# crowsonkb/style_transfer2

Hardware: AMD Instinct MI355X
Metric: style-transfer iters/sec @1024px VGG19 (higher is better)
Workload: dtype f32; 1 GPU; configs[1]: 1024x1024 single image per GPU, VGG19 to conv5_1, content conv4_2 + 5 style layers, adam fp32, 500 iterations per image; jobs=1, parallelism=independent jobs, 1 per GPU, no collective (replicas)

## Files before the change

style_transfer2_amd/csrc/gram.hip:

```cpp
#include "st2_kernels.h"
#include "env.h"
#include "wave_reduce.h"
#include <stdint.h>
#include <stdlib.h>

namespace st2 {

typedef float f32x16 __attribute__((ext_vector_type(16)));

constexpr int GKT = 32;
constexpr int GLD = GKT + 1;

GramPlan gram_plan(int C, int hw)
{
    GramPlan p;
    p.bt = C > 64 ? 128 : 64;
    const int t = (C + p.bt - 1) / p.bt;
    p.tiles = t * (t + 1) / 2;
    const int target128 = (int)env_int("ST2_GRAM_BLOCKS", 512), target64 = (int)env_int("ST2_GRAM_BLOCKS64", 1024);
    int want = p.bt == 128 ? target128 / p.tiles : (target64 + p.tiles - 1) / p.tiles;
    const int max_splits = (hw + 4 * GKT - 1) / (4 * GKT);
    if (want > max_splits) want = max_splits;
    if (want < 1) want = 1;
    int kslab = (hw + want - 1) / want;
// ... 88 lines not shown
            for (int i = 0; i < T; ++i)
#pragma unroll
                for (int j = 0; j < T; ++j)
                    acc[i][j] = __builtin_amdgcn_mfma_f32_32x32x2f32(av[i], bv[j], acc[i][j], 0, 0, 0);
        }
    }

    float* dst = slabs + (size_t)split * C * C;
#pragma unroll
    for (int i = 0; i < T; ++i)
#pragma unroll
        for (int j = 0; j < T; ++j) {
            const int col = j0 + wn * (T * 32) + j * 32 + l31;
#pragma unroll
            for (int e = 0; e < 16; ++e) {
                const int row = i0 + wm * (T * 32) + i * 32 + (e & 3) + 8 * (e >> 2) + 4 * khalf;
                if (row < C && col < C) dst[(size_t)row * C + col] = acc[i][j][e];
            }
        }
}

typedef __attribute__((address_space(3))) void* gram_lptr_t;
typedef float gf32x4 __attribute__((ext_vector_type(4)));

template <int BT>
__device__ __forceinline__ void gram_partial_dma_body(const float* __restrict__ F, unsigned f_bytes, float* __restrict__ slabs,
                                                      int C, int hw, int tiles_1d, int kslab)
{
    constexpr int T = BT / 64;
    constexpr int IMG = BT * 32;
    constexpr int PIECES = IMG / 256;
    constexpr int PPW = PIECES / 4;
    __shared__ __attribute__((aligned(16))) float smem[2][2][IMG];

    const int tid = threadIdx.x, lane = tid & 63;
    const int wave = __builtin_amdgcn_readfirstlane(tid >> 6);
    const int wm = wave >> 1, wn = wave & 1;
    const int n_ut = tiles_1d * (tiles_1d + 1) / 2;
    int tile = blockIdx.x % n_ut;
    const int split = blockIdx.x / n_ut;
    int ti = 0;
    while (tile >= tiles_1d - ti) { tile -= tiles_1d - ti; ++ti; }
    const int tj = ti + tile;
    const int i0 = ti * BT, j0 = tj * BT;
    const bool diag = ti == tj;
    const int kbeg = split * kslab;
    const int kend = min(hw, kbeg + kslab);
    const int nsteps = (kend - kbeg) / 32;

    const __amdgpu_buffer_rsrc_t rs = __builtin_amdgcn_make_buffer_rsrc((void*)F, 0, f_bytes, 0x00020000);
    unsigned aoff[PPW], boff[PPW];
#pragma unroll
    for (int t = 0; t < PPW; ++t) {
        const int slot = (wave + 4 * t) * 64 + lane;
        const int r = slot >> 3, q = (slot & 7) ^ ((r >> 1) & 7);
        aoff[t] = i0 + r < C ? ((unsigned)(i0 + r) * (unsigned)hw + (unsigned)kbeg + 4u * q) * 4u : 0xffffffffu;
        boff[t] = j0 + r < C ? ((unsigned)(j0 + r) * (unsigned)hw + (unsigned)kbeg + 4u * q) * 4u : 0xffffffffu;
    }
    auto dma = [&](int step, int stage) {
        const unsigned so = (unsigned)step * 128u;
#pragma unroll
        for (int t = 0; t < PPW; ++t) {
            __builtin_amdgcn_raw_ptr_buffer_load_lds(rs, (gram_lptr_t)(smem[stage][0] + (wave + 4 * t) * 256), 16,
                                                     aoff[t] == 0xffffffffu ? aoff[t] : aoff[t] + so, 0, 0, 0);
            if (!diag)
                __builtin_amdgcn_raw_ptr_buffer_load_lds(rs, (gram_lptr_t)(smem[stage][1] + (wave + 4 * t) * 256), 16,
                                                         boff[t] == 0xffffffffu ? boff[t] : boff[t] + so, 0, 0, 0);
        }
    };

    f32x16 acc[T][T];
#pragma unroll
    for (int i = 0; i < T; ++i)
#pragma unroll
        for (int j = 0; j < T; ++j)
#pragma unroll
            for (int e = 0; e < 16; ++e) acc[i][j][e] = 0.f;

    const int l31 = lane & 31;
    const bool hi = lane >= 32;
    int arow[T], brow[T];
#pragma unroll
    for (int i = 0; i < T; ++i) { arow[i] = wm * (T * 32) + i * 32 + l31; brow[i] = wn * (T * 32) + i * 32 + l31; }

    if (nsteps > 0) dma(0, 0);
    for (int st = 0; st < nsteps; ++st) {
        const int cur = st & 1;
        asm volatile("s_waitcnt vmcnt(0)" ::: "memory");
        __syncthreads();
        if (st + 1 < nsteps) dma(st + 1, cur ^ 1);
        const float* As = smem[cur][0];
        const float* Bs = diag ? smem[cur][0] : smem[cur][1];
#pragma unroll
        for (int q = 0; q < 8; ++q) {
            float a0[T], a1[T], b0[T], b1[T];
#pragma unroll
            for (int i = 0; i < T; ++i) {
                const gf32x4 v = *reinterpret_cast<const gf32x4*>(As + (arow[i] * 8 + (q ^ ((arow[i] >> 1) & 7))) * 4);
                a0[i] = hi ? v.y : v.x; a1[i] = hi ? v.w : v.z;
            }
#pragma unroll
            for (int j = 0; j < T; ++j) {
                const gf32x4 v = *reinterpret_cast<const gf32x4*>(Bs + (brow[j] * 8 + (q ^ ((brow[j] >> 1) & 7))) * 4);
                b0[j] = hi ? v.y : v.x; b1[j] = hi ? v.w : v.z;
            }
#pragma unroll
            for (int i = 0; i < T; ++i)
#pragma unroll
                for (int j = 0; j < T; ++j) {
                    acc[i][j] = __builtin_amdgcn_mfma_f32_32x32x2f32(a0[i], b0[j], acc[i][j], 0, 0, 0);
                    acc[i][j] = __builtin_amdgcn_mfma_f32_32x32x2f32(a1[i], b1[j], acc[i][j], 0, 0, 0);
                }
        }
    }

    const int khalf = lane >> 5;
    float* dst = slabs + (size_t)split * C * C;
#pragma unroll
    for (int i = 0; i < T; ++i)
#pragma unroll
        for (int j = 0; j < T; ++j) {
            const int col = j0 + wn * (T * 32) + j * 32 + l31;
#pragma unroll
            for (int e = 0; e < 16; ++e) {
                const int row = i0 + wm * (T * 32) + i * 32 + (e & 3) + 8 * (e >> 2) + 4 * khalf;
                if (row < C && col < C) dst[(size_t)row * C + col] = acc[i][j][e];
            }
        }
}

__global__ __launch_bounds__(256, 2) void gram_partial_dma_128(const float* F, unsigned f_bytes, float* slabs, int C, int hw, int tiles_1d, int kslab)
{ gram_partial_dma_body<128>(F, f_bytes, slabs, C, hw, tiles_1d, kslab); }
__global__ __launch_bounds__(256, 2) void gram_partial_dma_64(const float* F, unsigned f_bytes, float* slabs, int C, int hw, int tiles_1d, int kslab)
{ gram_partial_dma_body<64>(F, f_bytes, slabs, C, hw, tiles_1d, kslab); }

hipError_t launch_gram_partial(const float* F, float* slabs, int C, int hw, const GramPlan& pl, hipStream_t s,
                               const GramRoi* roi_in)
{
    const int t1 = (C + pl.bt - 1) / pl.bt;
    const unsigned grid = (unsigned)(pl.tiles * pl.splits);
    GramRoi roi = roi_in ? *roi_in : GramRoi{0, 0, hw, hw, (size_t)hw};
    if (!roi_in && !env_off("ST2_GRAM_DMA") && hw % 32 == 0 && pl.kslab % 32 == 0 && (reinterpret_cast<uintptr_t>(F) & 15) == 0 &&
        4ull * C * hw < 0xfffffff0ull) {
        const unsigned fb = (unsigned)(4ull * C * hw);
        if (pl.bt == 128) gram_partial_dma_128<<<grid, 256, 0, s>>>(F, fb, slabs, C, hw, t1, pl.kslab);
        else gram_partial_dma_64<<<grid, 256, 0, s>>>(F, fb, slabs, C, hw, t1, pl.kslab);
        return hipGetLastError();
    }
    if (pl.bt == 128) gram_partial_k<128><<<grid, 256, 0, s>>>(F, slabs, C, hw, t1, pl.kslab, roi);
    else gram_partial_k<64><<<grid, 256, 0, s>>>(F, slabs, C, hw, t1, pl.kslab, roi);
    return hipGetLastError();
}

__global__ __launch_bounds__(256) void gram_reduce_k(const float* __restrict__ slabs, const float* __restrict__ target,
                                                     float* __restrict__ out, float* __restrict__ partial,
                                                     int cc, int splits, float n, int C, int out_ld, int bt)
{
    __shared__ float scratch[4];
    float acc[1] = {0.f};
    for (int i = blockIdx.x * 256 + threadIdx.x; i < cc; i += gridDim.x * 256) {
        const int r = i / C, c = i - r * C;
        const int tr = r / bt, tc = c / bt;
        if (tr > tc) continue;
        float sum = 0.f;
        for (int s = 0; s < splits; ++s) sum += slabs[(size_t)s * cc + i];
        float v = sum / n;
        if (target) v -= target[i];
        out[r * out_ld + c] = v;
        acc[0] += v * v;
        if (tr < tc) { out[c * out_ld + r] = v; acc[0] += v * v; }
    }
    block_sum(acc, scratch);
    if (threadIdx.x == 0 && partial) partial[blockIdx.x] = acc[0];
}

__global__ __launch_bounds__(256) void gram_fold_k(const float* __restrict__ slabs, float* __restrict__ folded,
                                                   int cc, int splits, int per_group, int C, int bt)
{
    const int i = blockIdx.x * 256 + threadIdx.x;
    const int g = blockIdx.y;
    if (i >= cc) return;
    if ((i / C) / bt > (i % C) / bt) return;
    const int s0 = g * per_group, s1 = min(splits, s0 + per_group);
    float sum = 0.f;
    for (int s = s0; s < s1; ++s) sum += slabs[(size_t)s * cc + i];
    folded[(size_t)g * cc + i] = sum;
}

template <int GR_LANES>
__global__ __launch_bounds__(256) void gram_reduce_wide_k(const float* __restrict__ slabs, const float* __restrict__ target,
                                                          float* __restrict__ out, float* __restrict__ partial,
                                                          int cc, int splits, float n, int C, int out_ld, int bt)
{
    constexpr int GR_QUADS = 256 / GR_LANES, GR_ELEMS = 4 * GR_QUADS;
    __shared__ float4 part_s[GR_LANES][GR_QUADS];
    __shared__ float scratch[4];
    const int q = threadIdx.x % GR_QUADS, ln = threadIdx.x / GR_QUADS;
    float acc[1] = {0.f};
    for (int base = blockIdx.x * GR_ELEMS; base < cc; base += gridDim.x * GR_ELEMS) {
        const int i = base + 4 * q;
        const int r = i < cc ? i / C : 0, c = i < cc ? i - r * C : 0;
        const bool live = i < cc && r / bt <= c / bt;
        float4 sum = make_float4(0.f, 0.f, 0.f, 0.f);
        if (live)
            for (int s = ln; s < splits; s += GR_LANES) {
                const float4 v = *reinterpret_cast<const float4*>(slabs + (size_t)s * cc + i);
                sum.x += v.x; sum.y += v.y; sum.z += v.z; sum.w += v.w;
            }
        __syncthreads();
        part_s[ln][q] = sum;
        __syncthreads();
        if (ln == 0 && live) {
            float4 tot = part_s[0][q];
#pragma unroll
            for (int j = 1; j < GR_LANES; ++j) { const float4 p = part_s[j][q]; tot.x += p.x; tot.y += p.y; tot.z += p.z; tot.w += p.w; }
            float v[4] = {tot.x / n, tot.y / n, tot.z / n, tot.w / n};
            if (target) { const float4 t = *reinterpret_cast<const float4*>(target + i); v[0] -= t.x; v[1] -= t.y; v[2] -= t.z; v[3] -= t.w; }
            const bool mirror = r / bt < c / bt;
#pragma unroll
            for (int k = 0; k < 4; ++k) {
                out[r * out_ld + c + k] = v[k];
                acc[0] += v[k] * v[k];
                if (mirror) { out[(c + k) * out_ld + r] = v[k]; acc[0] += v[k] * v[k]; }
            }
        }
    }
    block_sum(acc, scratch);
    if (threadIdx.x == 0 && partial) partial[blockIdx.x] = acc[0];
}

int gram_fold_groups(const GramPlan& pl) { return pl.splits > 32 ? 32 : 0; }

hipError_t launch_gram_reduce(const float* slabs, float* folded, const float* target, float* out, int out_ld, float* partial,
                              int* n_partial, int C, double divisor, const GramPlan& pl, hipStream_t s)
{
    const int cc = C * C;
    int splits = pl.splits;
    if (splits > 32 && C % 4 == 0 && pl.bt % 4 == 0 && env_int("ST2_GRAM_REDUCE", 1) != 2) {
        const bool small = cc <= 128 * 128;
        const int grid = reduce_grid((size_t)cc, small ? 32 : 128, kMaxPartials);
        if (n_partial) *n_partial = grid;
        if (small) gram_reduce_wide_k<32><<<grid, 256, 0, s>>>(slabs, target, out, partial, cc, splits, (float)divisor, C, out_ld, pl.bt);
        else gram_reduce_wide_k<8><<<grid, 256, 0, s>>>(slabs, target, out, partial, cc, splits, (float)divisor, C, out_ld, pl.bt);
        return hipGetLastError();
    }
    const int groups = gram_fold_groups(pl);
    if (groups) {
        const int per = (pl.splits + groups - 1) / groups;
        gram_fold_k<<<dim3((cc + 255) / 256, groups), 256, 0, s>>>(slabs, folded, cc, pl.splits, per, C, pl.bt);
        slabs = folded;
        splits = (pl.splits + per - 1) / per;
    }
    const int grid = reduce_grid((size_t)cc, 256, kMaxPartials);
    if (n_partial) *n_partial = grid;
    gram_reduce_k<<<grid, 256, 0, s>>>(slabs, target, out, partial, cc, splits, (float)divisor, C, out_ld, pl.bt);
    return hipGetLastError();
}

}
```

style_transfer2_amd/csrc/passes.hip:

```cpp
#include "st2_kernels.h"
#include "channel_mean.h"
#include "wave_reduce.h"
#include <float.h>
#include <math.h>

namespace st2 {

int pooled_size(int n)
{
    int q = (n - 2 + 1) / 2;
    if (n - 2 < 0) q = 0;
    return q + 1;
}

__global__ __launch_bounds__(256) void maxpool_fwd_k(const float* __restrict__ in, float* __restrict__ out,
                                                     int C, int H, int W, int Ho, int Wo)
{
    const size_t total = (size_t)C * Ho * Wo;
    for (size_t idx = (size_t)blockIdx.x * 256 + threadIdx.x; idx < total; idx += (size_t)gridDim.x * 256) {
        const int px = (int)(idx % Wo);
        const int py = (int)((idx / Wo) % Ho);
        const int c = (int)(idx / ((size_t)Wo * Ho));
        const float* p = in + (size_t)c * H * W;
        const int r0 = 2 * py, c0 = 2 * px;
        float best = -FLT_MAX;
#pragma unroll
        for (int dr = 0; dr < 2; ++dr)
#pragma unroll
            for (int dc = 0; dc < 2; ++dc) {
                const int r = r0 + dr, cc = c0 + dc;
                if (r < H && cc < W) {
                    const float v = p[(size_t)r * W + cc];
                    if (v > best) best = v;
                }
            }
        out[idx] = best;
    }
}

__device__ __forceinline__ int first_max4(float a, float b, float c, float d, float* best)
{
    int arg = 0; float m = a;
    if (b > m) { m = b; arg = 1; }
    if (c > m) { m = c; arg = 2; }
    if (d > m) { m = d; arg = 3; }
    *best = m;
    return arg;
}

__global__ __launch_bounds__(256) void maxpool_fwd_v4_k(const float* __restrict__ in, float* __restrict__ out,
                                                        size_t n_patches, int W4, int Ho)
{
    for (size_t idx = (size_t)blockIdx.x * 256 + threadIdx.x; idx < n_patches; idx += (size_t)gridDim.x * 256) {
        const size_t q = idx % W4, pr = idx / W4;
        const float4 r0 = *reinterpret_cast<const float4*>(in + (pr * 2) * (size_t)W4 * 4 + q * 4);
        const float4 r1 = *reinterpret_cast<const float4*>(in + (pr * 2 + 1) * (size_t)W4 * 4 + q * 4);
        float2 o;
        first_max4(r0.x, r0.y, r1.x, r1.y, &o.x);
        first_max4(r0.z, r0.w, r1.z, r1.w, &o.y);
        *reinterpret_cast<float2*>(out + pr * (size_t)W4 * 2 + q * 2) = o;
    }
}

__global__ __launch_bounds__(256) void maxpool_bwd_v4_k(const float* __restrict__ dy, const float* __restrict__ x,
                                                        float* __restrict__ dx, const float* __restrict__ inject,
                                                        int apply_mask, size_t n_patches, int W4)
{
    for (size_t idx = (size_t)blockIdx.x * 256 + threadIdx.x; idx < n_patches; idx += (size_t)gridDim.x * 256) {
        const size_t q = idx % W4, pr = idx / W4;
        const size_t o0 = (pr * 2) * (size_t)W4 * 4 + q * 4, o1 = o0 + (size_t)W4 * 4;
        const float4 r0 = *reinterpret_cast<const float4*>(x + o0);
        const float4 r1 = *reinterpret_cast<const float4*>(x + o1);
        const float2 g = *reinterpret_cast<const float2*>(dy + pr * (size_t)W4 * 2 + q * 2);
        float best;
        const int a0 = first_max4(r0.x, r0.y, r1.x, r1.y, &best);
        const int a1 = first_max4(r0.z, r0.w, r1.z, r1.w, &best);
        float4 d0 = make_float4(a0 == 0 ? g.x : 0.f, a0 == 1 ? g.x : 0.f, a1 == 0 ? g.y : 0.f, a1 == 1 ? g.y : 0.f);
        float4 d1 = make_float4(a0 == 2 ? g.x : 0.f, a0 == 3 ? g.x : 0.f, a1 == 2 ? g.y : 0.f, a1 == 3 ? g.y : 0.f);
        if (apply_mask) {
            d0.x = r0.x > 0.f ? d0.x : 0.f; d0.y = r0.y > 0.f ? d0.y : 0.f; d0.z = r0.z > 0.f ? d0.z : 0.f; d0.w = r0.w > 0.f ? d0.w : 0.f;
            d1.x = r1.x > 0.f ? d1.x : 0.f; d1.y = r1.y > 0.f ? d1.y : 0.f; d1.z = r1.z > 0.f ? d1.z : 0.f; d1.w = r1.w > 0.f ? d1.w : 0.f;
        }
        if (inject) {
            const float4 i0 = *reinterpret_cast<const float4*>(inject + o0);
            const float4 i1 = *reinterpret_cast<const float4*>(inject + o1);
            d0.x += i0.x; d0.y += i0.y; d0.z += i0.z; d0.w += i0.w;
            d1.x += i1.x; d1.y += i1.y; d1.z += i1.z; d1.w += i1.w;
        }
        *reinterpret_cast<float4*>(dx + o0) = d0;
        *reinterpret_cast<float4*>(dx + o1) = d1;
    }
}

__global__ __launch_bounds__(256) void maxpool_bwd_amap_k(const float* __restrict__ dy, const unsigned char* __restrict__ amap,
                                                          float* __restrict__ dx, size_t n_patches, int W4)
{
    for (size_t idx = (size_t)blockIdx.x * 256 + threadIdx.x; idx < n_patches; idx += (size_t)gridDim.x * 256) {
        const size_t q = idx % W4, pr = idx / W4;
        const size_t o0 = (pr * 2) * (size_t)W4 * 4 + q * 4, o1 = o0 + (size_t)W4 * 4;
        const size_t po = pr * (size_t)W4 * 2 + q * 2;
        const float2 g = *reinterpret_cast<const float2*>(dy + po);
        const unsigned short mm = *reinterpret_cast<const unsigned short*>(amap + po);
        const unsigned m0 = mm & 0xffu, m1 = mm >> 8;
        const float g0 = (m0 & 4u) ? g.x : 0.f, g1 = (m1 & 4u) ? g.y : 0.f;
        const unsigned a0 = m0 & 3u, a1 = m1 & 3u;
        *reinterpret_cast<float4*>(dx + o0) = make_float4(a0 == 0 ? g0 : 0.f, a0 == 1 ? g0 : 0.f, a1 == 0 ? g1 : 0.f, a1 == 1 ? g1 : 0.f);
        *reinterpret_cast<float4*>(dx + o1) = make_float4(a0 == 2 ? g0 : 0.f, a0 == 3 ? g0 : 0.f, a1 == 2 ? g1 : 0.f, a1 == 3 ? g1 : 0.f);
    }
}

hipError_t launch_maxpool_bwd_amap(const float* dy, const unsigned char* amap, float* dx, int C, int H, int W, hipStream_t s)
{
    if (H % 2 != 0 || W % 4 != 0 || (reinterpret_cast<uintptr_t>(amap) & 1) != 0) return hipErrorInvalidValue;
    const size_t n_patches = (size_t)C * (H / 2) * (W / 4);
    maxpool_bwd_amap_k<<<reduce_grid(n_patches, 256, 65536), 256, 0, s>>>(dy, amap, dx, n_patches, W / 4);
    return hipGetLastError();
}

hipError_t launch_maxpool_fwd(const float* in, float* out, int C, int H, int W, hipStream_t s)
{
    const int Ho = pooled_size(H), Wo = pooled_size(W);
    const size_t total = (size_t)C * Ho * Wo;
    if (H % 2 == 0 && W % 4 == 0) {
        const size_t n_patches = (size_t)C * Ho * (W / 4);
        maxpool_fwd_v4_k<<<reduce_grid(n_patches, 256, 65536), 256, 0, s>>>(in, out, n_patches, W / 4, Ho);
        return hipGetLastError();
    }
    maxpool_fwd_k<<<reduce_grid(total, 256, 65536), 256, 0, s>>>(in, out, C, H, W, Ho, Wo);
    return hipGetLastError();
}

__global__ __launch_bounds__(256) void maxpool_bwd_k(const float* __restrict__ dy, const float* __restrict__ x,
                                                     float* __restrict__ dx, const float* __restrict__ inject,
                                                     int apply_mask, int C, int H, int W, int Ho, int Wo)
{
    const size_t total = (size_t)C * Ho * Wo;
    for (size_t idx = (size_t)blockIdx.x * 256 + threadIdx.x; idx < total; idx += (size_t)gridDim.x * 256) {
        const int px = (int)(idx % Wo);
        const int py = (int)((idx / Wo) % Ho);
        const int c = (int)(idx / ((size_t)Wo * Ho));
        const size_t base = (size_t)c * H * W;
        const int r0 = 2 * py, c0 = 2 * px;
        float best = -FLT_MAX;
        int arg = -1;
        float vals[4];
#pragma unroll
        for (int k = 0; k < 4; ++k) {
            const int r = r0 + (k >> 1), cc = c0 + (k & 1);
            vals[k] = 0.f;
            if (r < H && cc < W) {
                vals[k] = x[base + (size_t)r * W + cc];
                if (vals[k] > best) { best = vals[k]; arg = k; }
            }
        }
// ... 194 lines not shown
#pragma unroll
            for (int j = 0; j < 8; ++j) {
                v[0][j] = (__bf16)d0[j].x; v[1][j] = (__bf16)d0[j].y; v[2][j] = (__bf16)d0[j].z; v[3][j] = (__bf16)d0[j].w;
                v[4][j] = (__bf16)d1[j].x; v[5][j] = (__bf16)d1[j].y; v[6][j] = (__bf16)d1[j].z; v[7][j] = (__bf16)d1[j].w;
            }
            unsigned short* r0 = dx16 + (cb * hw + o0) * 8;
            unsigned short* r1 = dx16 + (cb * hw + o1) * 8;
#pragma unroll
            for (int k = 0; k < 4; ++k) {
                *reinterpret_cast<ap_bf16x8*>(r0 + k * 8) = v[k];
                *reinterpret_cast<ap_bf16x8*>(r1 + k * 8) = v[4 + k];
            }
        }
    }
}

hipError_t launch_avepool_bwd(const float* dy, const float* x, const float* inject, float* dx, unsigned short* dx16,
                              int C, int H, int W, hipStream_t s)
{
    if (!dx && !dx16) return hipErrorInvalidValue;
    const int Ho = pooled_size(H), Wo = pooled_size(W);
    const int CB = (C + 7) / 8;
    if (H % 2 == 0 && W % 4 == 0) {
        const size_t n_patches = (size_t)CB * Ho * (W / 4);
        avepool_bwd_v4_k<<<reduce_grid(n_patches, 256, 65536), 256, 0, s>>>(dy, x, inject, dx, dx16, C, W / 4, Ho, n_patches);
        return hipGetLastError();
    }
    const size_t total = (size_t)CB * H * W;
    avepool_bwd_k<<<reduce_grid(total, 256, 65536), 256, 0, s>>>(dy, x, inject, dx, dx16, C, H, W, Ho, Wo);
    return hipGetLastError();
}

__global__ __launch_bounds__(256) void layer_elem_k(const LayerElemArgs a)
{
    __shared__ float scratch[16];
    float acc[4] = {0.f, 0.f, 0.f, 0.f};
    float inv_c = 0.f, inv_d = 0.f;
    if (a.write) {
        if (a.content) inv_c = *a.norm_c;
        if (a.deepdream) inv_d = *a.norm_d;
    }
    const bool vec = !a.w && (a.n & 3) == 0 && ((reinterpret_cast<uintptr_t>(a.feat) | reinterpret_cast<uintptr_t>(a.inject) |
                                                 reinterpret_cast<uintptr_t>(a.target)) & 15) == 0;
    if (vec) {
        const size_t n4 = a.n >> 2;
        for (size_t q = (size_t)blockIdx.x * 256 + threadIdx.x; q < n4; q += (size_t)gridDim.x * 256) {
            const float4 f4 = reinterpret_cast<const float4*>(a.feat)[q];
            float4 t4 = make_float4(0.f, 0.f, 0.f, 0.f);
            if (a.content) t4 = reinterpret_cast<const float4*>(a.target)[q];
            const float fv[4] = {f4.x, f4.y, f4.z, f4.w}, tv[4] = {t4.x, t4.y, t4.z, t4.w};
            float ov[4];
#pragma unroll
            for (int j = 0; j < 4; ++j) {
                const float f = fv[j];
                float out = 0.f;
                if (a.content) {
                    const float d = f - tv[j];
                    const float gc = a.cn_coef * d;
                    acc[0] += d * d;
                    acc[1] += gc * gc;
                    if (a.write) out += (a.cw * gc) / inv_c;
                }
                if (a.deepdream) {
                    const float gd = a.dn_coef * f;
                    acc[2] += f * f;
                    acc[3] += gd * gd;
                    if (a.write) out += (a.dw * gd) / inv_d;
                }
                ov[j] = out;
            }
            if (a.write) reinterpret_cast<float4*>(a.inject)[q] = make_float4(ov[0], ov[1], ov[2], ov[3]);
        }
    } else
    for (size_t i = (size_t)blockIdx.x * 256 + threadIdx.x; i < a.n; i += (size_t)gridDim.x * 256) {
        if (a.w) {
            const int x = (int)(i % a.w), y = (int)((i / a.w) % a.h);
            if (y < a.ry0 || y >= a.ry1 || x < a.rx0 || x >= a.rx1) {
                if (a.write) a.inject[i] = 0.f;
                continue;
            }
        }
        const float f = a.feat[i];
        float out = 0.f;
        if (a.content) {
            const float d = f - a.target[i];
            const float gc = a.cn_coef * d;
            acc[0] += d * d;
            acc[1] += gc * gc;
            if (a.write) out += (a.cw * gc) / inv_c;
        }
        if (a.deepdream) {
            const float gd = a.dn_coef * f;
            acc[2] += f * f;
            acc[3] += gd * gd;
            if (a.write) out += (a.dw * gd) / inv_d;
        }
        if (a.write) a.inject[i] = out;
    }
    block_sum(acc, scratch);
    if (threadIdx.x == 0) {
        if (a.part_d2) a.part_d2[blockIdx.x] = acc[0];
        if (a.part_gc2) a.part_gc2[blockIdx.x] = acc[1];
        if (a.part_f2) a.part_f2[blockIdx.x] = acc[2];
        if (a.part_gd2) a.part_gd2[blockIdx.x] = acc[3];
    }
}

hipError_t launch_layer_elem(const LayerElemArgs& a, int* n_partial, hipStream_t s)
{
    const int grid = reduce_grid(a.n, 256 * 8, kMaxPartials);
    *n_partial = grid;
    layer_elem_k<<<grid, 256, 0, s>>>(a);
    return hipGetLastError();
}

__global__ __launch_bounds__(256) void finalize_norm_k(const float* part, int n_part, double n, float* norm)
{
    __shared__ double scratch[256];
    const double sum = sum_partials(part, n_part, scratch);
    if (threadIdx.x == 0) *norm = sqrtf((float)(sum / n));
}

hipError_t launch_finalize_norm(const float* partial, int n_partial, double n, float* norm, hipStream_t s)
{
    finalize_norm_k<<<1, 256, 0, s>>>(partial, n_partial, n, norm);
    return hipGetLastError();
}

__global__ __launch_bounds__(256) void scaled_accumulate_k(const float* __restrict__ S, float* __restrict__ inject,
                                                           float sw, const float* __restrict__ norm,
                                                           int accumulate, size_t n)
{
    const float coef = sw / *norm;
    for (size_t i = (size_t)blockIdx.x * 256 + threadIdx.x; i < n; i += (size_t)gridDim.x * 256) {
        const float base = accumulate ? inject[i] : 0.f;
        inject[i] = coef * S[i] + base;
    }
}

hipError_t launch_scaled_accumulate(const float* S, float* inject, float sw, const float* norm,
                                    int accumulate, size_t n, hipStream_t s)
{
    scaled_accumulate_k<<<reduce_grid(n, 256 * 4, 8192), 256, 0, s>>>(S, inject, sw, norm, accumulate, n);
    return hipGetLastError();
}

__device__ __forceinline__ float tv_k(float q, float half_beta, int beta_is_2)
{
    return beta_is_2 ? 1.0f : half_beta * powf(q, half_beta - 1.0f);
}

constexpr int IP_TY = 4, IP_TX = 256;
constexpr int IP_LW = IP_TX + 2;

__global__ __launch_bounds__(256) void image_pass_k(const ImagePassArgs a)
{
    __shared__ float scratch[32];
    __shared__ float u_s[(IP_TY + 2) * IP_LW];
    const int H = a.H, W = a.W, tid = threadIdx.x;
    const size_t plane = (size_t)H * W;
    const float half_beta = a.tv_beta * 0.5f;
    const int beta_is_2 = a.tv_beta == 2.0f;
    const float corr1 = a.dyn ? a.dyn[0] : a.corr1, corr2 = a.dyn ? a.dyn[1] : a.corr2, step = a.dyn ? a.dyn[2] : a.step;
    const int p_round = (int)a.p_pow;
    const int p_int = ((float)p_round == a.p_pow && p_round >= 1 && p_round <= 16) ? p_round : 0;
    const int tiles_x = (W + IP_TX - 1) / IP_TX, tiles_y = (H + IP_TY - 1) / IP_TY;
    const int n_tiles = a.C * tiles_y * tiles_x;
    float acc[6] = {0.f, 0.f, 0.f, 0.f, 0.f, 0.f};
    for (int tile = blockIdx.x; tile < n_tiles; tile += gridDim.x) {
        const int tx = tile % tiles_x, rest = tile / tiles_x;
        const int ty = rest % tiles_y, ch = rest / tiles_y;
        const int x0 = tx * IP_TX, y0 = ty * IP_TY;
        const float* p = a.x + (size_t)ch * plane;
        __syncthreads();
        for (int e = tid; e < (IP_TY + 2) * IP_LW; e += 256) {
            const int r = e / IP_LW, c = e - r * IP_LW;
            int gy = y0 - 1 + r, gx = x0 - 1 + c;
            gy = gy < 0 ? H - 1 : (gy >= H ? gy - H : gy);
            gx = gx < 0 ? W - 1 : (gx >= W ? gx - W : gx);
            u_s[e] = (gy < H && gx < W) ? p[(size_t)gy * W + gx] / 255.0f : 0.f;
        }
        __syncthreads();
        const int x = x0 + tid;
        if (x < W) {
#pragma unroll
            for (int ry = 0; ry < IP_TY; ++ry) {
                const int y = y0 + ry;
                if (y >= H) break;
                const float* us = u_s + (ry + 1) * IP_LW + tid + 1;
                const size_t idx = (size_t)ch * plane + (size_t)y * W + x;
                const float xv = a.x[idx];
                const float u = us[0];
                const float u_r = us[1], u_l = us[-1];
                const float u_d = us[IP_LW], u_u = us[-IP_LW];
                const float u_dl = us[IP_LW - 1], u_ur = us[-IP_LW + 1];
                const float a0 = u - u_r, b0 = u - u_d;
                const float q0 = (a0 * a0 + b0 * b0) + 1e-8f;
                const float k0 = tv_k(q0, half_beta, beta_is_2);
                const float da0 = (2.0f * a0) * k0, db0 = (2.0f * b0) * k0;
                const float aL = u_l - u, bL = u_l - u_dl;
                const float qL = (aL * aL + bL * bL) + 1e-8f;
                const float daL = (2.0f * aL) * tv_k(qL, half_beta, beta_is_2);
                const float aU = u_u - u_ur, bU = u_u - u;
                const float qU = (aU * aU + bU * bU) + 1e-8f;
                const float dbU = (2.0f * bU) * tv_k(qU, half_beta, beta_is_2);
                float g_tv = da0 + db0;
                g_tv -= daL;
                g_tv -= dbU;
                acc[0] += beta_is_2 ? q0 : powf(q0, half_beta);
                const float mag = fabsf(u);
                const float sgn = u > 0.f ? 1.f : (u < 0.f ? -1.f : 0.f);
                float pw, pw1;
                if (p_int) {
                    pw1 = p_int > 1 ? mag : 1.0f;
                    for (int k = 2; k < p_int; ++k) pw1 *= mag;
                    pw = pw1 * mag;
                } else {
                    pw = powf(mag, a.p_pow);
                    pw1 = powf(mag, a.p_pow - 1.0f);
                }
                acc[1] += pw;
                const float g_p = sgn * pw1;
                const float scd = a.scd ? a.scd[idx] : 0.f;
                const float tg = a.tv_w * g_tv;
                const float pg = a.p_w * g_p;
                float g = scd + tg;
                g += pg;
                acc[2] += scd * scd;
                acc[3] += tg * tg;
                acc[4] += pg * pg;
                acc[5] += g * g;
                if (a.grad) a.grad[idx] = g;
                if (a.x_out) {
                    const float m_old = a.m_is_zero ? 0.f : a.m[idx];
                    const float v_old = a.v_is_zero ? 0.f : a.v[idx];
                    const float m_new = a.d1 * m_old + a.c1 * g;
                    const float v_new = a.d2 * v_old + a.c2 * (g * g);
                    a.m[idx] = m_new;
                    a.v[idx] = v_new;
                    const float m_hat = m_new / corr1;
                    const float v_hat = v_new / corr2;
                    a.x_out[idx] = xv - (step * m_hat) / (sqrtf(v_hat) + 1e-8f);
                }
            }
        }
    }
    block_sum(acc, scratch);
    if (threadIdx.x == 0) {
#pragma unroll
        for (int i = 0; i < 6; ++i) a.partial[i * kMaxPartials + blockIdx.x] = acc[i];
    }
}

__global__ void set_scalars3_k(float* dst, float a, float b, float c) { dst[0] = a; dst[1] = b; dst[2] = c; }
hipError_t launch_set_scalars3(float* dst, float a, float b, float c, hipStream_t s)
{
    set_scalars3_k<<<1, 1, 0, s>>>(dst, a, b, c);
    return hipGetLastError();
}

hipError_t launch_image_pass(const ImagePassArgs& a, int* n_partial, hipStream_t s)
{
    const long long n_tiles = (long long)a.C * ((a.H + IP_TY - 1) / IP_TY) * ((a.W + IP_TX - 1) / IP_TX);
    const int grid = (int)(n_tiles < kMaxPartials ? (n_tiles < 1 ? 1 : n_tiles) : kMaxPartials);
    *n_partial = grid;
    image_pass_k<<<grid, 256, 0, s>>>(a);
    return hipGetLastError();
}

__global__ __launch_bounds__(256) void image_pass_tile_k(const ImageTileArgs t)
{
    __shared__ float scratch[32];
    const ImagePassArgs& a = t.base;
    const int th = t.th, tw = t.tw, ww = a.W;
    const size_t wplane = (size_t)a.H * a.W, tplane = (size_t)th * tw, rplane = (size_t)(th + 2) * (tw + 2);
    const size_t total = tplane * 3;
    const float half_beta = a.tv_beta * 0.5f;
    const int beta_is_2 = a.tv_beta == 2.0f;
    float acc[6] = {0.f, 0.f, 0.f, 0.f, 0.f, 0.f};
    for (size_t idx = (size_t)blockIdx.x * 256 + threadIdx.x; idx < total; idx += (size_t)gridDim.x * 256) {
        const int x = (int)(idx % tw);
        const int y = (int)((idx / tw) % th);
        const int c = (int)(idx / tplane);
        const float* p = a.x + c * wplane;
        const float* rg = t.ring + c * rplane;
        auto U = [&](int yy, int xx) -> float {
            const bool inside = yy >= 0 && yy < th && xx >= 0 && xx < tw;
            const float v = inside ? p[(size_t)(t.ty + yy) * ww + t.tx + xx] : rg[(size_t)(yy + 1) * (tw + 2) + xx + 1];
            return v / 255.0f;
        };
        const size_t widx = c * wplane + (size_t)(t.ty + y) * ww + t.tx + x;
        const float xv = p[(size_t)(t.ty + y) * ww + t.tx + x];
        const float u = xv / 255.0f;
        const float u_r = U(y, x + 1), u_d = U(y + 1, x), u_l = U(y, x - 1), u_u = U(y - 1, x);
        const float u_dl = U(y + 1, x - 1), u_ur = U(y - 1, x + 1);
        const float a0 = u - u_r, b0 = u - u_d;
        const float q0 = (a0 * a0 + b0 * b0) + 1e-8f;
        const float k0 = tv_k(q0, half_beta, beta_is_2);
        const float da0 = (2.0f * a0) * k0, db0 = (2.0f * b0) * k0;
        const float aL = u_l - u, bL = u_l - u_dl;
        const float qL = (aL * aL + bL * bL) + 1e-8f;
        const float daL = (2.0f * aL) * tv_k(qL, half_beta, beta_is_2);
        const float aU = u_u - u_ur, bU = u_u - u;
        const float qU = (aU * aU + bU * bU) + 1e-8f;
        const float dbU = (2.0f * bU) * tv_k(qU, half_beta, beta_is_2);
        float g_tv = da0 + db0;
        g_tv -= daL;
        g_tv -= dbU;
        acc[0] += beta_is_2 ? q0 : powf(q0, half_beta);
        const float mag = fabsf(u);
        const float sgn = u > 0.f ? 1.f : (u < 0.f ? -1.f : 0.f);
        acc[1] += powf(mag, a.p_pow);
        const float g_p = sgn * powf(mag, a.p_pow - 1.0f);
        const float scd = a.scd ? a.scd[widx] : 0.f;
        const float tg = a.tv_w * g_tv;
        const float pg = a.p_w * g_p;
        float g = scd + tg;
        g += pg;
        acc[2] += scd * scd;
        acc[3] += tg * tg;
        acc[4] += pg * pg;
        acc[5] += g * g;
        if (a.grad) a.grad[widx] = g;
        if (a.x_out) {
            const float m_old = a.m_is_zero ? 0.f : a.m[widx];
            const float v_old = a.v_is_zero ? 0.f : a.v[widx];
            const float m_new = a.d1 * m_old + a.c1 * g;
            const float v_new = a.d2 * v_old + a.c2 * (g * g);
            a.m[widx] = m_new;
            a.v[widx] = v_new;
            const float m_hat = m_new / a.corr1;
            const float v_hat = v_new / a.corr2;
            a.x_out[widx] = xv - (a.step * m_hat) / (sqrtf(v_hat) + 1e-8f);
        }
    }
    block_sum(acc, scratch);
    if (threadIdx.x == 0) {
#pragma unroll
        for (int i = 0; i < 6; ++i) a.partial[i * kMaxPartials + blockIdx.x] = acc[i];
    }
}

hipError_t launch_image_pass_tile(const ImageTileArgs& a, int* n_partial, hipStream_t s)
{
    const size_t total = (size_t)3 * a.th * a.tw;
    const int grid = reduce_grid(total, 256 * 4, kMaxPartials);
    *n_partial = grid;
    image_pass_tile_k<<<grid, 256, 0, s>>>(a);
    return hipGetLastError();
}

__global__ __launch_bounds__(256) void resample_h_k(const float* __restrict__ src, float* __restrict__ dst, size_t rows,
                                                    int w_in, int w_out, ResampleTable t, int clamp0)
{
    const size_t total = rows * w_out;
    for (size_t idx = (size_t)blockIdx.x * 256 + threadIdx.x; idx < total; idx += (size_t)gridDim.x * 256) {
        const int xx = (int)(idx % w_out);
        const size_t row = idx / w_out;
        const float* p = src + row * w_in + t.lo[xx];
        const double* k = t.k + (size_t)xx * t.kmax;
        double ss = 0.0;
        for (int i = 0; i < t.n[xx]; ++i) ss += (double)p[i] * k[i];
        float v = (float)ss;
        if (clamp0) v = v > 0.f ? v : 0.f;
        dst[idx] = v;
    }
}

__global__ __launch_bounds__(256) void resample_v_k(const float* __restrict__ src, float* __restrict__ dst, int planes,
                                                    int h_in, int h_out, int w, ResampleTable t, int clamp0)
{
    const size_t total = (size_t)planes * h_out * w;
    for (size_t idx = (size_t)blockIdx.x * 256 + threadIdx.x; idx < total; idx += (size_t)gridDim.x * 256) {
        const int x = (int)(idx % w);
        const int yy = (int)((idx / w) % h_out);
        const size_t pl = idx / ((size_t)w * h_out);
        const float* p = src + (pl * h_in + t.lo[yy]) * w + x;
        const double* k = t.k + (size_t)yy * t.kmax;
        double ss = 0.0;
        for (int i = 0; i < t.n[yy]; ++i) ss += (double)p[(size_t)i * w] * k[i];
        float v = (float)ss;
        if (clamp0) v = v > 0.f ? v : 0.f;
        dst[idx] = v;
    }
}

__global__ __launch_bounds__(256) void clamp0_copy_k(const float* src, float* dst, size_t n, int clamp0)
{
    for (size_t i = (size_t)blockIdx.x * 256 + threadIdx.x; i < n; i += (size_t)gridDim.x * 256)
        dst[i] = clamp0 ? (src[i] > 0.f ? src[i] : 0.f) : src[i];
}

hipError_t launch_resample(const float* src, float* tmp, float* dst, int planes, int h_in, int w_in, int h_out, int w_out,
                           const ResampleTable& tx, const ResampleTable& ty, int clamp0, hipStream_t s)
{
    const bool need_h = w_in != w_out, need_v = h_in != h_out;
    const float* cur = src;
    if (need_h) {
        float* out = need_v ? tmp : dst;
        const size_t rows = (size_t)planes * h_in;
        resample_h_k<<<reduce_grid(rows * w_out, 256, 16384), 256, 0, s>>>(cur, out, rows, w_in, w_out, tx, need_v ? 0 : clamp0);
        cur = out;
    }
    if (need_v) resample_v_k<<<reduce_grid((size_t)planes * h_out * w_out, 256, 16384), 256, 0, s>>>(cur, dst, planes, h_in, h_out, w_out, ty, clamp0);
    if (!need_h && !need_v) clamp0_copy_k<<<reduce_grid((size_t)planes * h_in * w_in, 1024, 8192), 256, 0, s>>>(src, dst, (size_t)planes * h_in * w_in, clamp0);
    return hipGetLastError();
}

template <typename T>
__global__ __launch_bounds__(256) void preprocess_k(const T* __restrict__ hwc, float* __restrict__ nchw, int H, int W)
{
    const size_t plane = (size_t)H * W;
    for (size_t i = (size_t)blockIdx.x * 256 + threadIdx.x; i < plane * 3; i += (size_t)gridDim.x * 256) {
        const int c = (int)(i / plane);
        const size_t p = i % plane;
        nchw[i] = (float)hwc[p * 3 + c] - kMean[c];
    }
}

// ... 176 lines not shown
```

Baseline: 143.7 it/s.

## Add float4 prefetching image pass kernel and batched loads in gram reduce

```diff
diff --git a/style_transfer2_amd/csrc/gram.hip b/style_transfer2_amd/csrc/gram.hip
--- a/style_transfer2_amd/csrc/gram.hip
+++ b/style_transfer2_amd/csrc/gram.hip
@@ -264,6 +264,9 @@
     return hipGetLastError();
 }
 
+constexpr int GR_BATCH = 8;
+
+template <bool BATCH>
 __global__ __launch_bounds__(256) void gram_reduce_k(const float* __restrict__ slabs, const float* __restrict__ target,
                                                      float* __restrict__ out, float* __restrict__ partial,
                                                      int cc, int splits, float n, int C, int out_ld, int bt)
@@ -275,6 +278,22 @@
         const int tr = r / bt, tc = c / bt;
         if (tr > tc) continue;
         float sum = 0.f;
+        if (BATCH) {
+            float v[GR_BATCH];
+            int s = 0;
+            for (; s + GR_BATCH <= splits; s += GR_BATCH) {
+#pragma unroll
+                for (int b = 0; b < GR_BATCH; ++b) v[b] = slabs[(size_t)(s + b) * cc + i];
+#pragma unroll
+                for (int b = 0; b < GR_BATCH; ++b) sum += v[b];
+            }
+            if (s < splits) {
+#pragma unroll
+                for (int b = 0; b < GR_BATCH; ++b) v[b] = slabs[(size_t)(s + b < splits ? s + b : s) * cc + i];
+#pragma unroll
+                for (int b = 0; b < GR_BATCH; ++b) if (s + b < splits) sum += v[b];
+            }
+        } else
         for (int s = 0; s < splits; ++s) sum += slabs[(size_t)s * cc + i];
         float v = sum / n;
         if (target) v -= target[i];
@@ -299,7 +318,7 @@
     folded[(size_t)g * cc + i] = sum;
 }
 
-template <int GR_LANES>
+template <int GR_LANES, bool BATCH>
 __global__ __launch_bounds__(256) void gram_reduce_wide_k(const float* __restrict__ slabs, const float* __restrict__ target,
                                                           float* __restrict__ out, float* __restrict__ partial,
                                                           int cc, int splits, float n, int C, int out_ld, int bt)
@@ -314,7 +333,26 @@
         const int r = i < cc ? i / C : 0, c = i < cc ? i - r * C : 0;
         const bool live = i < cc && r / bt <= c / bt;
         float4 sum = make_float4(0.f, 0.f, 0.f, 0.f);
-        if (live)
+        if (live && BATCH) {
+            float4 v[GR_BATCH];
+            int s = ln;
+            for (; s + (GR_BATCH - 1) * GR_LANES < splits; s += GR_BATCH * GR_LANES) {
+#pragma unroll
+                for (int b = 0; b < GR_BATCH; ++b) v[b] = *reinterpret_cast<const float4*>(slabs + (size_t)(s + b * GR_LANES) * cc + i);
+#pragma unroll
+                for (int b = 0; b < GR_BATCH; ++b) { sum.x += v[b].x; sum.y += v[b].y; sum.z += v[b].z; sum.w += v[b].w; }
+            }
+            if (s < splits) {
+#pragma unroll
+                for (int b = 0; b < GR_BATCH; ++b) {
+                    const int sb = s + b * GR_LANES;
+                    v[b] = *reinterpret_cast<const float4*>(slabs + (size_t)(sb < splits ? sb : s) * cc + i);
+                }
+#pragma unroll
+                for (int b = 0; b < GR_BATCH; ++b)
+                    if (s + b * GR_LANES < splits) { sum.x += v[b].x; sum.y += v[b].y; sum.z += v[b].z; sum.w += v[b].w; }
+            }
+        } else if (live)
             for (int s = ln; s < splits; s += GR_LANES) {
                 const float4 v = *reinterpret_cast<const float4*>(slabs + (size_t)s * cc + i);
                 sum.x += v.x; sum.y += v.y; sum.z += v.z; sum.w += v.w;
@@ -348,12 +386,14 @@
 {
     const int cc = C * C;
     int splits = pl.splits;
+    const bool batch = !env_off("ST2_GRAM_REDUCE_BATCH");
     if (splits > 32 && C % 4 == 0 && pl.bt % 4 == 0 && env_int("ST2_GRAM_REDUCE", 1) != 2) {
         const bool small = cc <= 128 * 128;
         const int grid = reduce_grid((size_t)cc, small ? 32 : 128, kMaxPartials);
         if (n_partial) *n_partial = grid;
-        if (small) gram_reduce_wide_k<32><<<grid, 256, 0, s>>>(slabs, target, out, partial, cc, splits, (float)divisor, C, out_ld, pl.bt);
-        else gram_reduce_wide_k<8><<<grid, 256, 0, s>>>(slabs, target, out, partial, cc, splits, (float)divisor, C, out_ld, pl.bt);
+        auto k = small ? (batch ? gram_reduce_wide_k<32, true> : gram_reduce_wide_k<32, false>)
+                       : (batch ? gram_reduce_wide_k<8, true> : gram_reduce_wide_k<8, false>);
+        k<<<grid, 256, 0, s>>>(slabs, target, out, partial, cc, splits, (float)divisor, C, out_ld, pl.bt);
         return hipGetLastError();
     }
     const int groups = gram_fold_groups(pl);
@@ -365,7 +405,8 @@
     }
     const int grid = reduce_grid((size_t)cc, 256, kMaxPartials);
     if (n_partial) *n_partial = grid;
-    gram_reduce_k<<<grid, 256, 0, s>>>(slabs, target, out, partial, cc, splits, (float)divisor, C, out_ld, pl.bt);
+    auto k = batch ? gram_reduce_k<true> : gram_reduce_k<false>;
+    k<<<grid, 256, 0, s>>>(slabs, target, out, partial, cc, splits, (float)divisor, C, out_ld, pl.bt);
     return hipGetLastError();
 }
 
diff --git a/style_transfer2_amd/csrc/passes.hip b/style_transfer2_amd/csrc/passes.hip
--- a/style_transfer2_amd/csrc/passes.hip
+++ b/style_transfer2_amd/csrc/passes.hip
@@ -1,5 +1,6 @@
 #include "st2_kernels.h"
 #include "channel_mean.h"
+#include "env.h"
 #include "wave_reduce.h"
 #include <float.h>
 #include <math.h>
@@ -607,12 +608,188 @@
     return hipGetLastError();
 }
 
+constexpr int IPV_TX = 256, IPV_C0 = 4, IPV_LW = IPV_C0 + IPV_TX + 4;
+constexpr int IPV_FLUSH = 8, IPV_MAX_FLUSH = 32;
+
+struct IpvStage { float4 xq, hq; float hs; };
+
+template <int TY>
+__global__ __launch_bounds__(64 * TY) void image_pass_vec_k(const ImagePassArgs a)
+{
+    __shared__ float scratch[32];
+    __shared__ __attribute__((aligned(16))) float u_s[(TY + 2) * IPV_LW];
+    const int H = a.H, W = a.W, tid = threadIdx.x, lx = tid & 63, ry = tid >> 6;
+    const size_t plane = (size_t)H * W;
+    const float half_beta = a.tv_beta * 0.5f;
+    const int beta_is_2 = a.tv_beta == 2.0f;
+    const float corr1 = a.dyn ? a.dyn[0] : a.corr1, corr2 = a.dyn ? a.dyn[1] : a.corr2, step = a.dyn ? a.dyn[2] : a.step;
+    const int p_round = (int)a.p_pow;
+    const int p_int = ((float)p_round == a.p_pow && p_round >= 1 && p_round <= 16) ? p_round : 0;
+    const int tiles_x = (W + IPV_TX - 1) / IPV_TX, tiles_y = (H + TY - 1) / TY;
+    const int n_tiles = a.C * tiles_y * tiles_x;
+    const int hl = tid - 64 * (TY - 1);
+    const bool halo_row = tid < 128, halo_col = hl >= 0 && hl < 2 * (TY + 2);
+    if (tid < 32) scratch[tid] = 0.f;
+    auto wrap_row = [&](int gy) { return gy < 0 ? H - 1 : (gy >= H ? gy - H : gy); };
+    auto fetch = [&](int tile, IpvStage& st) {
+        const int tx = tile % tiles_x, rest = tile / tiles_x;
+        const int ty = rest % tiles_y, ch = rest / tiles_y;
+        const int x0 = tx * IPV_TX, y0 = ty * TY, x = x0 + 4 * lx;
+        const float* p = a.x + (size_t)ch * plane;
+        st.xq = st.hq = make_float4(0.f, 0.f, 0.f, 0.f);
+        st.hs = 0.f;
+        const int gy = wrap_row(y0 + ry);
+        if (gy < H && x < W) st.xq = *reinterpret_cast<const float4*>(p + (size_t)gy * W + x);
+        if (halo_row) {
+            const int hy = wrap_row(tid < 64 ? y0 - 1 : y0 + TY);
+            if (hy < H && x < W) st.hq = *reinterpret_cast<const float4*>(p + (size_t)hy * W + x);
+        }
+        if (halo_col) {
+            const int sy = wrap_row(y0 - 1 + (hl >> 1));
+            const int sx = (hl & 1) ? (x0 + IPV_TX >= W ? 0 : x0 + IPV_TX) : (x0 == 0 ? W - 1 : x0 - 1);
+            if (sy < H) st.hs = p[(size_t)sy * W + sx];
+        }
+    };
+    float acc[6] = {0.f, 0.f, 0.f, 0.f, 0.f, 0.f}, hi[6] = {0.f, 0.f, 0.f, 0.f, 0.f, 0.f};
+    int in_acc = 0;
+    IpvStage st;
+    if ((int)blockIdx.x < n_tiles) fetch(blockIdx.x, st);
+    for (int tile = blockIdx.x; tile < n_tiles; tile += gridDim.x) {
+        const int tx = tile % tiles_x, rest = tile / tiles_x;
+        const int ty = rest % tiles_y, ch = rest / tiles_y;
+        const int x0 = tx * IPV_TX, y0 = ty * TY;
+        const int x = x0 + 4 * lx, y = y0 + ry;
+        const int cols = W - x0 < IPV_TX ? W - x0 : IPV_TX;
+        const bool live = y < H && x < W;
+        const size_t idx = (size_t)ch * plane + (size_t)(live ? y : 0) * W + (live ? x : 0);
+        float4 sq = make_float4(0.f, 0.f, 0.f, 0.f), mq = sq, vq = sq;
+        if (live) {
+            if (a.scd) sq = *reinterpret_cast<const float4*>(a.scd + idx);
+            if (a.x_out && !a.m_is_zero) mq = *reinterpret_cast<const float4*>(a.m + idx);
+            if (a.x_out && !a.v_is_zero) vq = *reinterpret_cast<const float4*>(a.v + idx);
+        }
+        const float4 xq = st.xq;
+        const float4 uq = make_float4(xq.x / 255.0f, xq.y / 255.0f, xq.z / 255.0f, xq.w / 255.0f);
+        float* row = u_s + (ry + 1) * IPV_LW + IPV_C0 + 4 * lx;
+        __syncthreads();
+        if (x < W) {
+            *reinterpret_cast<float4*>(row) = uq;
+            if (halo_row) {
+                const float4 h = st.hq;
+                *reinterpret_cast<float4*>(u_s + (tid < 64 ? 0 : TY + 1) * IPV_LW + IPV_C0 + 4 * lx) =
+                    make_float4(h.x / 255.0f, h.y / 255.0f, h.z / 255.0f, h.w / 255.0f);
+            }
+        }
+        if (halo_col) u_s[(hl >> 1) * IPV_LW + ((hl & 1) ? IPV_C0 + cols : IPV_C0 - 1)] = st.hs / 255.0f;
+        __syncthreads();
+        if (tile + (int)gridDim.x < n_tiles) fetch(tile + gridDim.x, st);
+        if (live) {
+            const float4 upq = *reinterpret_cast<const float4*>(row - IPV_LW), dnq = *reinterpret_cast<const float4*>(row + IPV_LW);
+            const float cur[6] = {row[-1], uq.x, uq.y, uq.z, uq.w, row[4]};
+            const float up[5] = {upq.x, upq.y, upq.z, upq.w, row[4 - IPV_LW]};
+            const float dn[5] = {row[IPV_LW - 1], dnq.x, dnq.y, dnq.z, dnq.w};
+            const float xv4[4] = {xq.x, xq.y, xq.z, xq.w}, scd4[4] = {sq.x, sq.y, sq.z, sq.w};
+            const float m4[4] = {mq.x, mq.y, mq.z, mq.w}, v4[4] = {vq.x, vq.y, vq.z, vq.w};
+            float g4[4], mn4[4], vn4[4], xn4[4];
+#pragma unroll
+            for (int j = 0; j < 4; ++j) {
+                const float xv = xv4[j];
+                const float u = cur[j + 1];
+                const float u_r = cur[j + 2], u_l = cur[j];
+                const float u_d = dn[j + 1], u_u = up[j];
+                const float u_dl = dn[j], u_ur = up[j + 1];
+                const float a0 = u - u_r, b0 = u - u_d;
+                const float q0 = (a0 * a0 + b0 * b0) + 1e-8f;
+                const float k0 = tv_k(q0, half_beta, beta_is_2);
+                const float da0 = (2.0f * a0) * k0, db0 = (2.0f * b0) * k0;
+                const float aL = u_l - u, bL = u_l - u_dl;
+                const float qL = (aL * aL + bL * bL) + 1e-8f;
+                const float daL = (2.0f * aL) * tv_k(qL, half_beta, beta_is_2);
+                const float aU = u_u - u_ur, bU = u_u - u;
+                const float qU = (aU * aU + bU * bU) + 1e-8f;
+                const float dbU = (2.0f * bU) * tv_k(qU, half_beta, beta_is_2);
+                float g_tv = da0 + db0;
+                g_tv -= daL;
+                g_tv -= dbU;
+                acc[0] += beta_is_2 ? q0 : powf(q0, half_beta);
+                const float mag = fabsf(u);
+                const float sgn = u > 0.f ? 1.f : (u < 0.f ? -1.f : 0.f);
+                float pw, pw1;
+                if (p_int) {
+                    pw1 = p_int > 1 ? mag : 1.0f;
+                    for (int k = 2; k < p_int; ++k) pw1 *= mag;
+                    pw = pw1 * mag;
+                } else {
+                    pw = powf(mag, a.p_pow);
+                    pw1 = powf(mag, a.p_pow - 1.0f);
+                }
+                acc[1] += pw;
+                const float g_p = sgn * pw1;
+                const float scd = scd4[j];
+                const float tg = a.tv_w * g_tv;
+                const float pg = a.p_w * g_p;
+                float g = scd + tg;
+                g += pg;
+                acc[2] += scd * scd;
+                acc[3] += tg * tg;
+                acc[4] += pg * pg;
+                acc[5] += g * g;
+                g4[j] = g;
+                if (a.x_out) {
+                    const float m_new = a.d1 * m4[j] + a.c1 * g;
+                    const float v_new = a.d2 * v4[j] + a.c2 * (g * g);
+                    mn4[j] = m_new;
+                    vn4[j] = v_new;
+                    const float m_hat = m_new / corr1;
+                    const float v_hat = v_new / corr2;
+                    xn4[j] = xv - (step * m_hat) / (sqrtf(v_hat) + 1e-8f);
+                }
+            }
+            if (a.grad) *reinterpret_cast<float4*>(a.grad + idx) = make_float4(g4[0], g4[1], g4[2], g4[3]);
+            if (a.x_out) {
+                *reinterpret_cast<float4*>(a.m + idx) = make_float4(mn4[0], mn4[1], mn4[2], mn4[3]);
+                *reinterpret_cast<float4*>(a.v + idx) = make_float4(vn4[0], vn4[1], vn4[2], vn4[3]);
+                *reinterpret_cast<float4*>(a.x_out + idx) = make_float4(xn4[0], xn4[1], xn4[2], xn4[3]);
+            }
+        }
+        if (++in_acc == IPV_FLUSH) {
+#pragma unroll
+            for (int i = 0; i < 6; ++i) { hi[i] += acc[i]; acc[i] = 0.f; }
+            in_acc = 0;
+        }
+    }
+#pragma unroll
+    for (int i = 0; i < 6; ++i) hi[i] += acc[i];
+    block_sum(hi, scratch);
+    if (threadIdx.x == 0) {
+#pragma unroll
+        for (int i = 0; i < 6; ++i) a.partial[i * kMaxPartials + blockIdx.x] = hi[i];
+    }
+}
+
+static int image_vec_rows(const ImagePassArgs& a)
+{
+    const long long mode = env_int("ST2_IMAGE_VEC", 1);
+    if (mode == 0 || a.W % 4 != 0 || a.C < 1 || a.H < 1 || a.W < 1) return 0;
+    const void* ptrs[] = {a.x, a.scd, a.grad, a.x_out, a.x_out ? a.m : nullptr, a.x_out ? a.v : nullptr};
+    for (const void* p : ptrs) if (reinterpret_cast<uintptr_t>(p) & 15) return 0;
+    const int tiles_x = (a.W + IPV_TX - 1) / IPV_TX;
+    const long long tiles4 = (long long)a.C * ((a.H + 3) / 4) * tiles_x, tiles2 = (long long)a.C * ((a.H + 1) / 2) * tiles_x;
+    const int rows = (mode == 2 || mode == 4) ? (int)mode : (tiles4 >= 512 ? 4 : 2);
+    if ((rows == 4 ? tiles4 : tiles2) > (long long)IPV_FLUSH * (IPV_MAX_FLUSH - 1) * kMaxPartials) return 0;
+    return rows;
+}
+
 hipError_t launch_image_pass(const ImagePassArgs& a, int* n_partial, hipStream_t s)
 {
-    const long long n_tiles = (long long)a.C * ((a.H + IP_TY - 1) / IP_TY) * ((a.W + IP_TX - 1) / IP_TX);
+    const int rows = image_vec_rows(a);
+    const int ty = rows ? rows : IP_TY;
+    const long long n_tiles = (long long)a.C * ((a.H + ty - 1) / ty) * ((a.W + IP_TX - 1) / IP_TX);
     const int grid = (int)(n_tiles < kMaxPartials ? (n_tiles < 1 ? 1 : n_tiles) : kMaxPartials);
     *n_partial = grid;
-    image_pass_k<<<grid, 256, 0, s>>>(a);
+    if (rows == 4) image_pass_vec_k<4><<<grid, 256, 0, s>>>(a);
+    else if (rows == 2) image_pass_vec_k<2><<<grid, 128, 0, s>>>(a);
+    else image_pass_k<<<grid, 256, 0, s>>>(a);
     return hipGetLastError();
 }
 
```

Measured after the change: 144.2 it/s, median of 6. No clear change (+0.3%).

## Prefetch next image tile into registers and load halo with float4 quads

Applied to the files above, without the earlier changes.

```diff
diff --git a/style_transfer2_amd/csrc/passes.hip b/style_transfer2_amd/csrc/passes.hip
--- a/style_transfer2_amd/csrc/passes.hip
+++ b/style_transfer2_amd/csrc/passes.hip
@@ -500,11 +500,15 @@
 
 constexpr int IP_TY = 4, IP_TX = 256;
 constexpr int IP_LW = IP_TX + 2;
-
+constexpr int IP_SLOTS = (IP_TY + 2) * IP_LW;
+constexpr int IP_NRAW = (IP_SLOTS + 255) / 256;
+static_assert(IP_TY == 4 && IP_TX == 256 && IP_NRAW <= 9, "the quad mapping: 64 quads per row, 6 rows over 256 + 128 threads");
+
+template <bool QUADS>
 __global__ __launch_bounds__(256) void image_pass_k(const ImagePassArgs a)
 {
     __shared__ float scratch[32];
-    __shared__ float u_s[(IP_TY + 2) * IP_LW];
+    __shared__ float u_s[IP_SLOTS];
     const int H = a.H, W = a.W, tid = threadIdx.x;
     const size_t plane = (size_t)H * W;
     const float half_beta = a.tv_beta * 0.5f;
@@ -514,22 +518,103 @@
     const int p_int = ((float)p_round == a.p_pow && p_round >= 1 && p_round <= 16) ? p_round : 0;
     const int tiles_x = (W + IP_TX - 1) / IP_TX, tiles_y = (H + IP_TY - 1) / IP_TY;
     const int n_tiles = a.C * tiles_y * tiles_x;
+    const bool adam = a.x_out != nullptr;
+    const bool load_m = adam && !a.m_is_zero, load_v = adam && !a.v_is_zero;
+    const int hr = (tid - 128) >> 1, hside = tid & 1;
+
+    const int q4 = 4 * (tid & 63);
+    auto quad_src = [&](int k, int x0, int y0, int nx, int nr) -> long long {
+        const int r = (tid >> 6) + 4 * k;
+        int gy = y0 - 1 + r;
+        gy = gy < 0 ? H - 1 : (gy >= H ? gy - H : gy);
+        return (r < nr && q4 < nx) ? (long long)gy * W + x0 + q4 : -1;
+    };
+    auto side_src = [&](int x0, int y0, int nx, int nr) -> long long {
+        int gy = y0 - 1 + hr, gx = hside ? x0 + nx : x0 - 1;
+        gy = gy < 0 ? H - 1 : (gy >= H ? gy - H : gy);
+        gx = gx < 0 ? W - 1 : (gx >= W ? gx - W : gx);
+        return (tid >= 128 && hr < nr) ? (long long)gy * W + gx : -1;
+    };
+    auto slot_src = [&](int k, int x0, int y0) -> long long {
+        const int e = tid + 256 * k;
+        const int r = e / IP_LW, c = e - r * IP_LW;
+        int gy = y0 - 1 + r, gx = x0 - 1 + c;
+        gy = gy < 0 ? H - 1 : (gy >= H ? gy - H : gy);
+        gx = gx < 0 ? W - 1 : (gx >= W ? gx - W : gx);
+        return (e < IP_SLOTS && gy < H && gx < W) ? (long long)gy * W + gx : -1;
+    };
+
+    float4 rq[2];
+    float rs[IP_NRAW];
+    auto request = [&](int tile, bool on) {
+        const int tx = tile % tiles_x, rest = tile / tiles_x;
+        const int ty = rest % tiles_y, ch = rest / tiles_y;
+        const int x0 = tx * IP_TX, y0 = ty * IP_TY;
+        const float* p = a.x + (on ? (size_t)ch * plane : 0);
+        if constexpr (QUADS) {
+            const int nx = min(IP_TX, W - x0), nr = min(IP_TY, H - y0) + 2;
+#pragma unroll
+            for (int k = 0; k < 2; ++k) {
+                const long long o = quad_src(k, x0, y0, nx, nr);
+                rq[k] = *reinterpret_cast<const float4*>(p + ((o < 0 || !on) ? 0 : o));
+            }
+            const long long o = side_src(x0, y0, nx, nr);
+            rs[0] = p[(o < 0 || !on) ? 0 : o];
+        } else {
+#pragma unroll
+            for (int k = 0; k < IP_NRAW; ++k) {
+                const long long o = slot_src(k, x0, y0);
+                rs[k] = p[(o < 0 || !on) ? 0 : o];
+            }
+        }
+    };
+    auto publish = [&](int tile) {
+        const int tx = tile % tiles_x, ty = (tile / tiles_x) % tiles_y;
+        const int x0 = tx * IP_TX, y0 = ty * IP_TY;
+        if constexpr (QUADS) {
+            const int nx = min(IP_TX, W - x0), nr = min(IP_TY, H - y0) + 2;
+#pragma unroll
+            for (int k = 0; k < 2; ++k)
+                if (quad_src(k, x0, y0, nx, nr) >= 0) {
+                    float* us = u_s + ((tid >> 6) + 4 * k) * IP_LW + 1 + q4;
+                    us[0] = rq[k].x / 255.0f; us[1] = rq[k].y / 255.0f; us[2] = rq[k].z / 255.0f; us[3] = rq[k].w / 255.0f;
+                }
+            if (side_src(x0, y0, nx, nr) >= 0) u_s[hr * IP_LW + (hside ? nx + 1 : 0)] = rs[0] / 255.0f;
+        } else {
+#pragma unroll
+            for (int k = 0; k < IP_NRAW; ++k) {
+                const int e = tid + 256 * k;
+                if (e < IP_SLOTS) u_s[e] = slot_src(k, x0, y0) >= 0 ? rs[k] / 255.0f : 0.f;
+            }
+        }
+    };
+    const float* scd_p = a.scd ? a.scd : a.x;
+    const float* m_p = load_m ? a.m : a.x;
+    const float* v_p = load_v ? a.v : a.x;
+
     float acc[6] = {0.f, 0.f, 0.f, 0.f, 0.f, 0.f};
+    request(blockIdx.x, (int)blockIdx.x < n_tiles);
     for (int tile = blockIdx.x; tile < n_tiles; tile += gridDim.x) {
         const int tx = tile % tiles_x, rest = tile / tiles_x;
         const int ty = rest % tiles_y, ch = rest / tiles_y;
         const int x0 = tx * IP_TX, y0 = ty * IP_TY;
-        const float* p = a.x + (size_t)ch * plane;
+        const int x = x0 + tid;
+        float xv_r[IP_TY], scd_r[IP_TY], m_r[IP_TY], v_r[IP_TY];
+#pragma unroll
+        for (int ry = 0; ry < IP_TY; ++ry) {
+            const size_t idx = (x < W && y0 + ry < H) ? (size_t)ch * plane + (size_t)(y0 + ry) * W + x : 0;
+            xv_r[ry] = a.x[idx];
+            scd_r[ry] = scd_p[idx];
+            m_r[ry] = m_p[idx];
+            v_r[ry] = v_p[idx];
+        }
         __syncthreads();
-        for (int e = tid; e < (IP_TY + 2) * IP_LW; e += 256) {
-            const int r = e / IP_LW, c = e - r * IP_LW;
-            int gy = y0 - 1 + r, gx = x0 - 1 + c;
-            gy = gy < 0 ? H - 1 : (gy >= H ? gy - H : gy);
-            gx = gx < 0 ? W - 1 : (gx >= W ? gx - W : gx);
-            u_s[e] = (gy < H && gx < W) ? p[(size_t)gy * W + gx] / 255.0f : 0.f;
-        }
+        publish(tile);
         __syncthreads();
-        const int x = x0 + tid;
+        {
+            const int next = tile + (int)gridDim.x;
+            request(next < n_tiles ? next : tile, next < n_tiles);
+        }
         if (x < W) {
 #pragma unroll
             for (int ry = 0; ry < IP_TY; ++ry) {
@@ -537,7 +622,7 @@
                 if (y >= H) break;
                 const float* us = u_s + (ry + 1) * IP_LW + tid + 1;
                 const size_t idx = (size_t)ch * plane + (size_t)y * W + x;
-                const float xv = a.x[idx];
+                const float xv = xv_r[ry];
                 const float u = us[0];
                 const float u_r = us[1], u_l = us[-1];
                 const float u_d = us[IP_LW], u_u = us[-IP_LW];
@@ -569,7 +654,7 @@
                 }
                 acc[1] += pw;
                 const float g_p = sgn * pw1;
-                const float scd = a.scd ? a.scd[idx] : 0.f;
+                const float scd = a.scd ? scd_r[ry] : 0.f;
                 const float tg = a.tv_w * g_tv;
                 const float pg = a.p_w * g_p;
                 float g = scd + tg;
@@ -580,8 +665,8 @@
                 acc[5] += g * g;
                 if (a.grad) a.grad[idx] = g;
                 if (a.x_out) {
-                    const float m_old = a.m_is_zero ? 0.f : a.m[idx];
-                    const float v_old = a.v_is_zero ? 0.f : a.v[idx];
+                    const float m_old = a.m_is_zero ? 0.f : m_r[ry];
+                    const float v_old = a.v_is_zero ? 0.f : v_r[ry];
                     const float m_new = a.d1 * m_old + a.c1 * g;
                     const float v_new = a.d2 * v_old + a.c2 * (g * g);
                     a.m[idx] = m_new;
@@ -612,7 +697,8 @@
     const long long n_tiles = (long long)a.C * ((a.H + IP_TY - 1) / IP_TY) * ((a.W + IP_TX - 1) / IP_TX);
     const int grid = (int)(n_tiles < kMaxPartials ? (n_tiles < 1 ? 1 : n_tiles) : kMaxPartials);
     *n_partial = grid;
-    image_pass_k<<<grid, 256, 0, s>>>(a);
+    if ((a.W & 3) == 0 && (reinterpret_cast<uintptr_t>(a.x) & 15) == 0) image_pass_k<true><<<grid, 256, 0, s>>>(a);
+    else image_pass_k<false><<<grid, 256, 0, s>>>(a);
     return hipGetLastError();
 }
 
```

Result: no change. 143.5 it/s before, 143.9 it/s after, median of 6 (+0.2%).
